# MarioPasc/MU-Diff

Hardware: AMD Instinct MI355X
Metric: 256x256 slices/sec (4-step dual-gen reverse) (higher is better)
Workload: dtype f32 (convs/attention: fp16 hi+lo split MFMA x3; 3x3 convs that fill the chip: fp16 hi.hi + e4m3 cross terms; fp32 accumulate); 1 GPU; BASELINE config 3 (BraTS-shaped test-split batches of 32; model and slice shapes of config 2): 4-step dual-generator sampling, 256x256, nf=64, ch_mult 1-2-4, 32 slices per GPU per step, batch-sharded over 1 GPU(s), weights replicated; batch=32, hipgraph=True

## Files before the change

include/mudiff_hip.h:

```cpp
#ifndef MUDIFF_HIP_H
#define MUDIFF_HIP_H

#include <stdint.h>

#ifdef __cplusplus
extern "C" {
#endif

#define MUD_OK 0
#define MUD_ERR_ARG 1
#define MUD_ERR_LAUNCH 2
#define MUD_ERR_UNSUPPORTED 3

#define MUD_ACT_NONE 0
#define MUD_ACT_SIGMOID 1
#define MUD_ACT_TANH 2
#define MUD_ACT_SILU 3
#define MUD_ACT_LRELU 4

#define MUD_PRO_NONE 0
#define MUD_PRO_AFFINE 1
#define MUD_PRO_AFFINE_SILU 2
#define MUD_PRO_LRELU 3

// ... 42 lines not shown
  const float* x;  int B, H, W, Cin, ldx;
  const void* w;   int64_t w_bstride;
  int ks, stride, pad;
  const float* pro_scale; const float* pro_shift; int pro_ld; int pro_mode;
  const float* bias;
  const float* bias2; int bias2_ld;
  const float* res; int ldr;
  float out_scale; int act;
  const float* emul; int ld_emul;
  const float* egate; int ld_egate;
  const float* eother; int ld_eother;
  float* out; int Cout, ldo;
  int sub2;
  double* stats; int stats_ld;
  int emul_cout;
  const double* gn_sums; int gn_sums_ld;
  int gn_G; float gn_eps; double gn_count;
  const float* gn_gamma; const float* gn_beta;
  int64_t gn_bstride;
  void* splitk_ws; int64_t splitk_ws_bytes;
  unsigned* splitk_counters; int splitk_ncounters;
  const void* skip_w; const float* skip_bias; float* skip_out; int skip_ldo;
  int prec; int w_exp;
} mud_conv_args;

int mud_conv2d_direct(const mud_conv_args* a, void* stream);

int64_t mud_packed_weight_bytes(int ks, int Cin, int Cout);
int mud_pack_weights(const float* src, int64_t s_tap, int64_t s_ci, int64_t s_co, int64_t src_bstride,
                     int ks, int Cin, int Cout, int nbatch, void* dst, void* stream);
int mud_pack_weights_prec(const float* src, int64_t s_tap, int64_t s_ci, int64_t s_co, int64_t src_bstride,
                          int ks, int Cin, int Cout, int nbatch, int prec, int w_exp, void* dst, void* stream);
int64_t mud_packed_weight_bytes_prec(int ks, int Cin, int Cout, int prec);
int mud_conv2d_mfma(const mud_conv_args* a, void* stream);
int mud_conv2d_mfma_prec_supported(const mud_conv_args* a, int prec);
int64_t mud_conv2d_mfma_splitk_bytes(const mud_conv_args* a);

typedef struct mud_census_args {
  const float* x; int B, H, W, C, ldx;
  const float* pro_scale; const float* pro_shift; int pro_ld; int pro_mode;
} mud_census_args;
typedef struct mud_census_out {
  uint64_t n, n_over, n_under, n_fp16_over, amax_bits;
} mud_census_out;
int mud_e4m3_census(const mud_census_args* a, mud_census_out* out, void* stream);

int mud_upfirdn2d(const float* in, int64_t planes, int H, int W, const float* kernel, int kh, int kw,
                  int up_x, int up_y, int down_x, int down_y, int pad_x0, int pad_x1, int pad_y0, int pad_y1,
                  float* out, void* stream);
int mud_fir_nhwc(const float* x, int B, int H, int W, int C, int ldx, const float* kernel_host, int kh, int kw,
                 int up, int down, int pad0, int pad1,
                 const float* pro_scale, const float* pro_shift, int pro_ld, int pro_mode,
                 float* out_h, int ldh, float* out_x, int ldxo, void* stream);

int mud_minibatch_stddev(const float* x, int B, int64_t hw, int C, int ld, int group, float* out, void* stream);

int mud_attention_supported(int C);
int64_t mud_attention_ws_bytes(int B, int N, int C);
int mud_attention(const float* qkv, int B, int N, int C, int ld, float scale, float* out, int ldo, void* ws, void* stream);
// ... 112 lines not shown
```

mu-diff_amd/backbones/layerspp.py:

```python
import numpy as np
import torch
import torch.nn as nn

from mudiff_hip import ops, precision
from mudiff_hip.ops import (ACT_NONE, ACT_SILU, INV_SQRT2, PRO_AFFINE, PRO_AFFINE_SILU, View)

from . import dense_layer, layers, up_or_down_sampling

conv1x1 = layers.ddpm_conv1x1
conv3x3 = layers.ddpm_conv3x3
NIN = layers.NIN
default_init = layers.default_init
dense = dense_layer.dense

FIR_K = (1, 3, 3, 1)


def _groups(c):
    return min(c // 4, 32)


def use_mfma(cin, cout):
    return cin % 4 == 0 and cin >= 8

# ... 268 lines not shown
            self.Conv_2 = conv1x1(in_ch, out_ch)
        self.skip_rescale, self.act, self.in_ch, self.out_ch = skip_rescale, act, in_ch, out_ch
        self.dropout = dropout

    def _prepare(self):
        d = dict(c0=ConvParam(self.Conv_0), c1=ConvParam(self.Conv_1))
        if hasattr(self, 'Conv_2'):
            d['c2'] = ConvParam(self.Conv_2)
            if self.up:
                d['c2'].bias = None
                d['c1'].bias = (self.Conv_1.bias.detach() + self.Conv_2.bias.detach()).contiguous()
        return d

    def run(self, x: View, style0, style1, tbias, out: View = None, arena=None):
        if self.dropout and self.training:
            raise NotImplementedError('dropout > 0 in training mode is not part of the inference path')
        p = self.prepared()
        fused = False
        gn0 = self.GroupNorm_0.scale_shift(x, style0)
        sc0, sh0 = (gn0, None) if isinstance(gn0, ops.LazyGN) else gn0
        if self.up:
            kk, up, down, pad = up_or_down_sampling.fir_params('up' if self.fir else 'naive_up', self.fir_kernel)
            h_in, _ = ops.fir_nhwc(x, kk, up, down, pad, pro=(sc0, sh0, PRO_AFFINE_SILU), want_h=True, want_x=False)
            x_skip, _ = ops.fir_nhwc(p['c2'](x), kk, up, down, pad)
            h = p['c0'](h_in, bias2=tbias, arena=arena)
        elif self.down:
            kk, up, down, pad = up_or_down_sampling.fir_params('down' if self.fir else 'naive_down', self.fir_kernel)
            h_in, x_skip = ops.fir_nhwc(x, kk, up, down, pad, pro=(sc0, sh0, PRO_AFFINE_SILU), want_h=True, want_x=True)
            h = p['c0'](h_in, bias2=tbias, arena=arena)
        else:
            x_skip = x
            fused = 'c2' in p and p['c0'].mfma and p['c2'].mfma and ops.fused_skip_ok(x, self.out_ch, PRO_AFFINE_SILU)
            if fused:
                x_skip = View.empty(x.B, x.H, x.W, self.out_ch, x.device)
                h = p['c0'](x, pro=(sc0, sh0, PRO_AFFINE_SILU), bias2=tbias, arena=arena, skip=(p['c2'].w, p['c2'].bias, x_skip))
            else:
                h = p['c0'](x, pro=(sc0, sh0, PRO_AFFINE_SILU), bias2=tbias, arena=arena)
        gn1 = self.GroupNorm_1.scale_shift(h, style1)
        sc1, sh1 = (gn1, None) if isinstance(gn1, ops.LazyGN) else gn1
        if 'c2' in p and not self.up and not fused:
            x_skip = p['c2'](x_skip)
        return p['c1'](h, pro=(sc1, sh1, PRO_AFFINE_SILU), res=x_skip, out_scale=INV_SQRT2 if self.skip_rescale else 1.0, out=out)

    def forward(self, x, temb=None, zemb=None):
        st0 = ops.dense(zemb, self.GroupNorm_0.style.weight.detach(), self.GroupNorm_0.style.bias.detach())
        st1 = ops.dense(zemb, self.GroupNorm_1.style.weight.detach(), self.GroupNorm_1.style.bias.detach())
        tb = None
        if temb is not None:
            tb = ops.dense(temb, self.Dense_0.weight.detach(), self.Dense_0.bias.detach(), act_in=ACT_SILU)
        return self.run(View.from_nchw(x), st0, st1, tb).to_nchw()


class ConvFeatBlock(nn.Module, _Prepared):

    def __init__(self, act, in_ch=None, out_ch=None, zemb_dim=256):
        super().__init__()
        self.conv1 = conv3x3(in_ch, out_ch)
        self.group_norm = GroupNorm_Conv(min(out_ch // 4, 32), out_ch)
        self.act = act
        self.conv2 = conv3x3(out_ch, out_ch)

    def _prepare(self):
        return dict(c1=ConvParam(self.conv1), c2=ConvParam(self.conv2))

    def run(self, x: View, out: View = None, arena=None):
# ... 124 lines not shown
```

mu-diff_amd/csrc/conv_direct.hip:

```cpp
#include "mud_common.h"
#include <stdlib.h>

template <int VO, int VI>
__global__ __launch_bounds__(256) void k_conv_direct(mud_conv_args a, int Ho, int Wo, int co_groups) {
  extern __shared__ __attribute__((aligned(16))) char smem_raw[];
  float* st_lds = (float*)smem_raw;
  const int b = blockIdx.y;
  if (a.stats) {
    for (int i = threadIdx.x; i < 2 * a.Cout; i += 256) st_lds[i] = 0.f;
    __syncthreads();
  }
  const unsigned total = (unsigned)Ho * (unsigned)Wo * (unsigned)co_groups;
  const unsigned nthreads = gridDim.x * blockDim.x;
  const unsigned stride = (nthreads / (unsigned)co_groups) * (unsigned)co_groups;
  const unsigned first = blockIdx.x * blockDim.x + threadIdx.x;
  const int cg = (int)(first % (unsigned)co_groups);
  float ssum[VO], ssq[VO];
#pragma unroll
  for (int j = 0; j < VO; ++j) ssum[j] = ssq[j] = 0.f;
  for (uint64_t idx64 = first; first < stride && idx64 < total; idx64 += stride) {
    const unsigned p = (unsigned)idx64 / (unsigned)co_groups;
    const int oy = (int)(p / (unsigned)Wo);
    const int ox = (int)(p - (unsigned)oy * (unsigned)Wo);
    const int co = cg * VO;
// ... 198 lines not shown
  }
  const int gy = ty0 + py, gx = tx0 + px;
  if (gy < a.H && gx < a.W) {
    const int64_t opix = ((int64_t)b * a.H + gy) * a.W + gx;
#pragma unroll
    for (int j = 0; j < COUT; ++j) {
      float v = acc[j];
      if (a.bias) v += a.bias[j];
      if (a.res) v += a.res[opix * a.ldr + j];
      a.out[opix * a.ldo + j] = mud_act(v * a.out_scale, a.act);
    }
  }
}

extern "C" int mud_conv2d_direct(const mud_conv_args* ap, void* stream) {
  MUD_REQUIRE(ap, "mud_conv2d_direct: null args");
  const mud_conv_args a = *ap;
  MUD_REQUIRE(a.x && a.w && a.out, "mud_conv2d_direct: null pointer");
  MUD_REQUIRE(a.B >= 0 && a.H > 0 && a.W > 0 && a.Cin > 0 && a.Cout > 0 && a.ks >= 1 && a.stride >= 1 && a.pad >= 0,
              "mud_conv2d_direct: bad sizes");
  MUD_REQUIRE(a.ldx >= a.Cin && a.ldo >= a.Cout, "mud_conv2d_direct: ld smaller than C");
  MUD_REQUIRE(a.pro_mode == MUD_PRO_NONE || a.pro_mode == MUD_PRO_LRELU || (a.pro_scale && a.pro_shift && a.pro_ld >= a.Cin), "mud_conv2d_direct: prologue arrays missing");
  MUD_REQUIRE(!a.res || a.ldr >= a.Cout, "mud_conv2d_direct: bad residual view");
  const int Ho = (a.H + 2 * a.pad - a.ks) / a.stride + 1, Wo = (a.W + 2 * a.pad - a.ks) / a.stride + 1;
  MUD_REQUIRE(Ho > 0 && Wo > 0, "mud_conv2d_direct: empty output");
  if (a.B == 0) return MUD_OK;
  const bool vo4 = a.Cout % 4 == 0 && a.ldo % 4 == 0 && mud_aligned16(a.out) && mud_aligned16(a.w) && (a.w_bstride % 16 == 0);
  const bool vi4 = a.Cin % 4 == 0 && a.ldx % 4 == 0 && mud_aligned16(a.x);
  const int co_groups = vo4 ? a.Cout / 4 : a.Cout;
  if (a.Cin == 1 && a.ks == 3 && ((a.stride == 1 && a.pad == 1) || (a.stride == 2 && a.pad == 0)) && vo4 && !a.emul && !a.egate && co_groups <= 256 && a.pro_mode == MUD_PRO_NONE && a.w_bstride == 0 &&
      (!a.res || (a.ldr % 4 == 0 && mud_aligned16(a.res))) && (!a.bias || mud_aligned16(a.bias)) &&
      (!a.bias2 || (a.bias2_ld % 4 == 0 && mud_aligned16(a.bias2)))) {
    MUD_REQUIRE(a.B <= 65535 && (!a.stats || a.stats_ld >= a.Cout), "mud_conv2d_direct: bad batch / stats view");
    const int spb = 256 / co_groups, strips_per_row = (int)mud_cdiv(Wo, HEAD_PIX);
    int64_t blocks = mud_cdiv((int64_t)Ho * strips_per_row, spb);
    if (blocks > 256 * 16) blocks = 256 * 16;
    if (a.stats) {
      static const int cap = getenv("MUD_HEAD_CAP") ? atoi(getenv("MUD_HEAD_CAP")) : 0;
      int64_t per_image = 2048 / a.B > 16 ? 2048 / a.B : 16;
      const int64_t lim = cap > 0 ? cap : (a.B == 1 ? 256 : 128);
      if (per_image > lim) per_image = lim;
      if (blocks > per_image) blocks = per_image;
    }
    if (a.stride == 1)
      hipLaunchKernelGGL(k_conv_head3x3<1>, dim3((int)blocks, a.B), dim3(256), a.stats ? 2 * a.Cout * sizeof(float) : 0, (hipStream_t)stream, a, co_groups,
                         strips_per_row, Ho, Wo);
// ... 38 lines not shown
```

mu-diff_amd/csrc/conv_mfma.hip:

```cpp
#include "mud_common.h"
#include <stdlib.h>
#include <type_traits>
#include <utility>

typedef int i32x4 __attribute__((ext_vector_type(4)));
typedef int i32x8 __attribute__((ext_vector_type(8)));
typedef _Float16 f16x4 __attribute__((ext_vector_type(4)));
typedef _Float16 f16x8 __attribute__((ext_vector_type(8)));

typedef mud_h16x4 h16x4;
typedef mud_h16x8 h16x8;
__device__ __forceinline__ int cm_e4m3x4(f32x4 v, float scale) {
  v = v * scale;
#pragma unroll
  for (int e = 0; e < 4; ++e) v[e] = __builtin_amdgcn_fmed3f(v[e], -448.0f, 448.0f);
  int p = __builtin_amdgcn_cvt_pk_fp8_f32(v[0], v[1], 0, false);
  return __builtin_amdgcn_cvt_pk_fp8_f32(v[2], v[3], p, true);
}
#define CM_BN 64
#define CM_BPLANE (CM_BN * 32)
#define CM_BSTEP (2 * CM_BPLANE)
#define CM_PIX 80
#define CM_GN_MAXC 1024
#define CM_GN_BYTES (2 * CM_GN_MAXC * 4)
// ... 312 lines not shown
        if (DUAL) acc2[m][n][i] = 0.f;
      }
  const int lane_a2 = ((wm * MT) * 32 + r) * 64 + ((hh ^ ((r >> 2) & 3)) << 4);

  if constexpr (X8) {
    if (q == 0) {
#pragma unroll
      for (int j = 0; j < G::NLOAD; ++j) {
        *(i32x4*)(smem + loff[j] + 64) = i32x4{0, 0, 0, 0};
        *(i32x4*)(smem + G::BUF + loff[j] + 64) = i32x4{0, 0, 0, 0};
      }
    }
  }
  dma_b(kc0 * G::NG);
  dma_b2(kc0);
  fetch_raw(kc0);

  const int emul_lim = a.emul_cout > 0 ? a.emul_cout : a.Cout;
  const bool vec = ((a.Cout | a.ldo | emul_lim | (a.res ? a.ldr : 0) | (a.emul ? a.ld_emul : 0) | (a.egate ? (a.ld_egate | a.ld_eother) : 0)) & 3) == 0 &&
                   mud_dev_aligned16(a.out) && (!a.res || mud_dev_aligned16(a.res)) && (!a.emul || mud_dev_aligned16(a.emul)) &&
                   (!a.egate || (mud_dev_aligned16(a.egate) && mud_dev_aligned16(a.eother)));
  const bool slab_mode = KS == 3 && nsplit > 1 && fin.counters != nullptr;
  const bool res_in_acc = !DUAL && KS == 3 && a.res != nullptr && !a.sub2 && nsplit == 1;
  if (res_in_acc) {
#pragma unroll
    for (int n = 0; n < 2; ++n) {
      const int co = (nt * WN + wn) * CM_BN + n * 32 + r;
#pragma unroll
      for (int m = 0; m < MT; ++m) {
        const int gy = ty0 + wm * MT + m;
#pragma unroll
        for (int reg = 0; reg < 16; ++reg) {
          const int gx = tx0 + (reg & 3) + 8 * (reg >> 2) + 4 * hh;
          const bool ok = gy < a.H && gx < a.W && co < a.Cout;
          acc[m][n][reg] = ok ? a.res[(((int64_t)b * a.H + gy) * a.W + gx) * a.ldr + co] : 0.f;
        }
      }
    }
  }

  if (gn_fold) {
    cm_gn_to_lds(a, b, tid, G::NT, (float*)(smem + G::GN_OFF), gn_c);
    __syncthreads();
  } else if (PRO == MUD_PRO_AFFINE || PRO == MUD_PRO_AFFINE_SILU) {
    float* sc_lds = (float*)(smem + G::GN_OFF);
    for (int c = tid; c < a.Cin; c += G::NT) {
      sc_lds[c] = psc[c];
// ... 831 lines not shown
      return MUD_ERR_LAUNCH;
    }
    attr_once.ok();
  }
  const int k16s = (int)mud_cdiv(a.Cin, 16), ntiles = (int)mud_cdiv(a.Cout, CM_BN * WN);
  const int lds = G::lds_bytes((PRO == MUD_PRO_AFFINE || PRO == MUD_PRO_AFFINE_SILU) ? a.Cin : 0);
  int tiles_x = 1;
  int64_t tiles;
  if (KS == 3) {
    tiles_x = (int)mud_cdiv(a.W, 32);
    tiles = (int64_t)tiles_x * mud_cdiv(a.H, WM * MT);
  } else {
    tiles = mud_cdiv((int64_t)a.H * a.W, G::P);
  }
  int64_t nblocks = tiles * ntiles * a.B;
  MUD_REQUIRE(nblocks <= 0x7fffffff, "mud_conv2d_mfma: grid too large");
  if constexpr (KS == 3) {
    const int64_t npix = (int64_t)a.B * a.H * a.W;
    int ns = 1;
    static const bool two_launches = getenv("MUD_CONV_SPLITK_2LAUNCH") != nullptr;
    const bool in_launch = !two_launches && a.splitk_counters && nblocks <= a.splitk_ncounters;
    if ((!DUAL || in_launch) && a.splitk_ws && mud_aligned16(a.splitk_ws) && cm_split_eligible(a)) ns = cm_splits(nblocks, k16s);
    if (ns > 1 && a.splitk_ws_bytes < cm_slab_bytes(ns, nblocks, 64 * WM * WN * 32 * MT * (DUAL ? 2 : 1))) ns = 1;
    if (ns > 1) {
      mud_conv_args p = a;
      p.out = (float*)a.splitk_ws;
      p.ldo = a.Cout;
      p.bias = p.bias2 = p.res = nullptr;
      p.out_scale = 1.0f;
      p.act = MUD_ACT_NONE;
      p.stats = nullptr;
      const int64_t stride = npix * a.Cout;
      if (in_launch) {
        hipLaunchKernelGGL((k_conv_mfma<KS, MT, WM, WN, PRO, DUAL, PREC>), dim3((unsigned)(nblocks * ns)), dim3(64 * WM * WN), lds, s, a, tiles_x,
                           (int)tiles, ntiles, k16s, (unsigned)(nblocks * ns), ns, (int64_t)0, CmFin{(float*)a.splitk_ws, a.splitk_counters});
        MUD_CHECK_LAUNCH("mud_conv2d_mfma(split-K, reduced in the launch)");
        return MUD_OK;
      }
      hipLaunchKernelGGL((k_conv_mfma<KS, MT, WM, WN, PRO, DUAL, PREC>), dim3((unsigned)(nblocks * ns)), dim3(64 * WM * WN), lds, s, p, tiles_x,
                         (int)tiles, ntiles, k16s, (unsigned)(nblocks * ns), ns, stride, CmFin{nullptr, nullptr});
      MUD_CHECK_LAUNCH("mud_conv2d_mfma(split-K)");
      const int64_t HW = (int64_t)a.H * a.W;
      int ppb = 32;
      while (ppb > 1 && HW % ppb) ppb >>= 1;
      hipLaunchKernelGGL(k_splitk_epilogue, dim3((unsigned)mud_cdiv(npix, ppb)), dim3(256), 0, s, a, (const float*)a.splitk_ws, ns, stride, a.Cout,
                         npix, ppb);
// ... 36 lines not shown
  if (!no8x1r && !a.skip_w && ntiles == 1 && a.Cin <= 64 && a.H >= 8 && blocks2 >= 512) v = CMV_8X1R, nb = blocks2;
  else if (ntiles % 2 == 0 && a.H >= 8 && blocks8 >= 256) v = CMV_8X2, nb = blocks8;
  else if (!no16 && a.H >= 16 && blocks16 >= 256) v = CMV_16X1, nb = blocks16;
  else if (blocks2 >= 512 && a.H >= 8) v = CMV_MT2, nb = blocks2;
  else v = CMV_MT1, nb = mud_cdiv(a.W, 32) * mud_cdiv(a.H, 4) * ntiles * a.B;
  if (blocks) *blocks = nb;
  return v;
}

extern "C" int64_t mud_conv2d_mfma_splitk_bytes(const mud_conv_args* ap) {
  if (!ap || ap->ks != 3 || ap->B <= 0 || ap->H <= 0 || ap->W <= 0 || ap->Cin <= 0 || ap->Cout <= 0 || !cm_split_eligible(*ap)) return 0;
  int64_t blocks = 0;
  int v = cm_variant3(*ap, &blocks);
  if (ap->skip_w) {
    if (!ap->splitk_counters) return 0;
    if (v != CMV_8X2 && v != CMV_16X1) {
      v = CMV_MT1;
      blocks = mud_cdiv(ap->W, 32) * mud_cdiv(ap->H, 4) * mud_cdiv(ap->Cout, CM_BN) * ap->B;
    }
  }
  const int ns = cm_splits(blocks, (int)mud_cdiv(ap->Cin, 16));
  const int tile_words = ((v == CMV_8X2 || v == CMV_16X1) ? 512 * 64 : v == CMV_MT2 ? 256 * 64 : v == CMV_8X1R ? 512 * 32 : 256 * 32) * (ap->skip_w ? 2 : 1);
  return ns > 1 ? cm_slab_bytes(ns, blocks, tile_words) : 0;
}

static bool cm_fp8x_built(const mud_conv_args& a) {
  if (a.ks != 3 || a.sub2 || (a.pro_mode != MUD_PRO_NONE && a.pro_mode != MUD_PRO_AFFINE_SILU)) return false;
  if (a.skip_w && a.pro_mode != MUD_PRO_AFFINE_SILU) return false;
  const int v = cm_variant3(a, nullptr);
  return v == CMV_8X2 || v == CMV_16X1 || v == CMV_8X1R;
}
extern "C" int mud_conv2d_mfma_prec_supported(const mud_conv_args* ap, int prec) {
  if (!ap || ap->B <= 0 || ap->H <= 0 || ap->W <= 0 || ap->Cin <= 0 || ap->Cout <= 0) return 0;
  if (prec == MUD_PREC_16X3) return ap->ks == 1 || ap->ks == 3;
  if (prec == MUD_PREC_16X1)
    return ap->ks == 3 && ap->pro_mode >= MUD_PRO_NONE && ap->pro_mode <= MUD_PRO_LRELU && (!ap->skip_w || ap->pro_mode == MUD_PRO_AFFINE_SILU);
  mud_conv_args a = *ap;
  a.prec = prec;
  return prec == MUD_PREC_FP8X && cm_fp8x_built(a);
}

extern "C" int mud_conv2d_mfma(const mud_conv_args* ap, void* stream) {
  MUD_REQUIRE(ap, "mud_conv2d_mfma: null args");
  mud_conv_args a = *ap;
  MUD_REQUIRE(a.x && a.w && a.out, "mud_conv2d_mfma: null pointer");
  MUD_REQUIRE((a.ks == 1 || a.ks == 3) && a.stride == 1 && a.pad == a.ks / 2, "mud_conv2d_mfma: only ks in {1,3}, stride 1, pad ks/2 (got ks=%d stride=%d pad=%d)", a.ks, a.stride, a.pad);
// ... 10 lines not shown
  if ((a.pro_mode == MUD_PRO_AFFINE || a.pro_mode == MUD_PRO_AFFINE_SILU) && a.gn_sums) {
    MUD_REQUIRE(a.Cin <= CM_GN_MAXC && a.gn_G > 0 && a.Cin % a.gn_G == 0 && a.gn_sums_ld >= a.Cin && a.gn_count > 0,
                "mud_conv2d_mfma: folded GroupNorm needs Cin <= %d, Cin %% gn_G == 0, gn_sums_ld >= Cin, gn_count > 0 (Cin=%d gn_G=%d)", CM_GN_MAXC, a.Cin, a.gn_G);
    MUD_REQUIRE((a.gn_gamma == nullptr) == (a.gn_beta == nullptr) && a.gn_bstride >= 0, "mud_conv2d_mfma: folded GroupNorm: gamma and beta come together");
    a.pro_scale = a.pro_shift = a.x;
    a.pro_ld = 0;
  } else if (a.pro_mode == MUD_PRO_AFFINE || a.pro_mode == MUD_PRO_AFFINE_SILU) {
    a.gn_sums = nullptr;
    MUD_REQUIRE(a.pro_scale && a.pro_shift && a.pro_ld >= a.Cin && a.pro_ld % 4 == 0 && mud_aligned16(a.pro_scale) && mud_aligned16(a.pro_shift),
                "mud_conv2d_mfma: prologue arrays missing or misaligned");
    MUD_REQUIRE(a.Cin <= CM_GN_MAXC, "mud_conv2d_mfma: a launch with prologue arrays takes Cin <= %d (the kernels keep them in LDS; Cin=%d)", CM_GN_MAXC, a.Cin);
  } else {
    a.pro_scale = a.pro_shift = a.x;
    a.pro_ld = 0;
    a.gn_sums = nullptr;
  }
  if (a.skip_w) {
    MUD_REQUIRE(a.ks == 3 && a.pro_mode == MUD_PRO_AFFINE_SILU && !a.res && !a.sub2 && !a.emul && !a.egate,
                "mud_conv2d_mfma: the fused skip conv needs ks == 3, the AFFINE_SILU prologue and a plain epilogue");
    MUD_REQUIRE(a.skip_out && a.Cin <= 512 && a.Cout % 4 == 0 && a.skip_ldo >= a.Cout && a.skip_ldo % 4 == 0 && a.ldo % 4 == 0 &&
                mud_aligned16(a.skip_w) && mud_aligned16(a.skip_out) && mud_aligned16(a.out),
                "mud_conv2d_mfma: fused skip conv needs Cin <= 512, Cout %% 4 == 0 and aligned float4 output rows (Cin=%d Cout=%d)", a.Cin, a.Cout);
  }
  MUD_REQUIRE(a.prec == MUD_PREC_16X3 || a.prec == MUD_PREC_FP8X || a.prec == MUD_PREC_16X1, "mud_conv2d_mfma: unknown arithmetic plan prec=%d", a.prec);
  MUD_REQUIRE(a.prec != MUD_PREC_16X1 || a.ks == 3, "mud_conv2d_mfma: MUD_PREC_16X1 is built for ks == 3 only (got ks=%d)", a.ks);
  MUD_REQUIRE(a.prec != MUD_PREC_FP8X || (cm_fp8x_built(a) && a.w_exp >= -100 && a.w_exp <= 100),
              "mud_conv2d_mfma: MUD_PREC_FP8X is not built for this launch (ask mud_conv2d_mfma_prec_supported first; the weights were packed for it and cannot be read by another plan)");
  if (a.B == 0) return MUD_OK;
  hipStream_t s = (hipStream_t)stream;
#ifdef MUD_EXPERIMENT_WS
  if (cm_ws_wanted(a)) return cm_ws_dispatch(a, s);
#endif
  if (a.prec == MUD_PREC_FP8X) {
    const int v8 = cm_variant3(a, nullptr);
    if (v8 == CMV_8X1R) return a.pro_mode == MUD_PRO_NONE ? cm_launch_pro<3, 1, 8, 1, MUD_PRO_NONE, false, MUD_PREC_FP8X>(a, s) : cm_launch_pro<3, 1, 8, 1, MUD_PRO_AFFINE_SILU, false, MUD_PREC_FP8X>(a, s);
    const bool x2 = v8 == CMV_8X2;
    if (a.skip_w) return x2 ? cm_launch_pro<3, 2, 4, 2, MUD_PRO_AFFINE_SILU, true, MUD_PREC_FP8X>(a, s) : cm_launch_pro<3, 2, 8, 1, MUD_PRO_AFFINE_SILU, true, MUD_PREC_FP8X>(a, s);
    if (a.pro_mode == MUD_PRO_NONE) return x2 ? cm_launch_pro<3, 2, 4, 2, MUD_PRO_NONE, false, MUD_PREC_FP8X>(a, s) : cm_launch_pro<3, 2, 8, 1, MUD_PRO_NONE, false, MUD_PREC_FP8X>(a, s);
    return x2 ? cm_launch_pro<3, 2, 4, 2, MUD_PRO_AFFINE_SILU, false, MUD_PREC_FP8X>(a, s) : cm_launch_pro<3, 2, 8, 1, MUD_PRO_AFFINE_SILU, false, MUD_PREC_FP8X>(a, s);
  }
  if (a.prec == MUD_PREC_16X1) {
    constexpr int P1 = MUD_PREC_16X1;
    if (a.skip_w) {
      switch (cm_variant3(a, nullptr)) {
        case CMV_8X2: return cm_launch_pro<3, 2, 4, 2, MUD_PRO_AFFINE_SILU, true, P1>(a, s);
        case CMV_16X1: return cm_launch_pro<3, 2, 8, 1, MUD_PRO_AFFINE_SILU, true, P1>(a, s);
// ... 36 lines not shown
```

mu-diff_amd/mudiff_hip/__init__.py:

```python
from __future__ import annotations

import ctypes as C
import os

import torch

_HERE = os.path.dirname(os.path.abspath(__file__))
_SHIPPED = os.path.join(_HERE, 'libmudiff_hip.so')
_LIB_PATH = os.environ.get('MUDIFF_HIP_LIB', _SHIPPED)
_lib = None
PREC_16X3, PREC_FP8X, PREC_16X1 = 0, 1, 2

ACT_NONE, ACT_SIGMOID, ACT_TANH, ACT_SILU, ACT_LRELU = 0, 1, 2, 3, 4
PRO_NONE, PRO_AFFINE, PRO_AFFINE_SILU, PRO_LRELU = 0, 1, 2, 3


class MudiffHipError(RuntimeError):
    pass


class ConvArgs(C.Structure):
    _fields_ = [
        ('x', C.c_void_p), ('B', C.c_int), ('H', C.c_int), ('W', C.c_int), ('Cin', C.c_int), ('ldx', C.c_int),
        ('w', C.c_void_p), ('w_bstride', C.c_int64),
        ('ks', C.c_int), ('stride', C.c_int), ('pad', C.c_int),
        ('pro_scale', C.c_void_p), ('pro_shift', C.c_void_p), ('pro_ld', C.c_int), ('pro_mode', C.c_int),
        ('bias', C.c_void_p),
        ('bias2', C.c_void_p), ('bias2_ld', C.c_int),
        ('res', C.c_void_p), ('ldr', C.c_int),
        ('out_scale', C.c_float), ('act', C.c_int),
        ('emul', C.c_void_p), ('ld_emul', C.c_int), ('egate', C.c_void_p), ('ld_egate', C.c_int), ('eother', C.c_void_p), ('ld_eother', C.c_int),
        ('out', C.c_void_p), ('Cout', C.c_int), ('ldo', C.c_int),
        ('sub2', C.c_int),
        ('stats', C.c_void_p), ('stats_ld', C.c_int),
        ('emul_cout', C.c_int),
        ('gn_sums', C.c_void_p), ('gn_sums_ld', C.c_int), ('gn_G', C.c_int), ('gn_eps', C.c_float), ('gn_count', C.c_double),
        ('gn_gamma', C.c_void_p), ('gn_beta', C.c_void_p), ('gn_bstride', C.c_int64),
        ('splitk_ws', C.c_void_p), ('splitk_ws_bytes', C.c_int64),
        ('splitk_counters', C.c_void_p), ('splitk_ncounters', C.c_int),
        ('skip_w', C.c_void_p), ('skip_bias', C.c_void_p), ('skip_out', C.c_void_p), ('skip_ldo', C.c_int),
        ('prec', C.c_int), ('w_exp', C.c_int),
    ]


MLP_MAX_LAYERS = 6


class MlpArgs(C.Structure):
    _fields_ = [
        ('x', C.c_void_p), ('ldx', C.c_int), ('B', C.c_int),
        ('nlayers', C.c_int), ('dims', C.c_int * (MLP_MAX_LAYERS + 1)),
        ('W', C.c_void_p * MLP_MAX_LAYERS), ('b', C.c_void_p * MLP_MAX_LAYERS),
        ('pixel_norm', C.c_int), ('act', C.c_int), ('act_last', C.c_int),
        ('out', C.c_void_p), ('ldo', C.c_int), ('maxdim', C.c_int),
    ]


class CensusArgs(C.Structure):
    _fields_ = [
        ('x', C.c_void_p), ('B', C.c_int), ('H', C.c_int), ('W', C.c_int), ('C', C.c_int), ('ldx', C.c_int),
        ('pro_scale', C.c_void_p), ('pro_shift', C.c_void_p), ('pro_ld', C.c_int), ('pro_mode', C.c_int),
    ]


# ... 15 lines not shown
_SIGNATURES = {
    'mud_version': (C.c_int, []),
    'mud_last_error': (C.c_char_p, []),
    'mud_build_flags': (C.c_char_p, []),
    'mud_posterior_sample': (_I, [_P, _P, _P, _P, _P, _P, _P, _P, _I, _P, _I, _L, _P]),
    'mud_q_sample': (_I, [_P, _P, _P, _I, _P, _P, _I, _P, _I, _L, _P]),
    'mud_timestep_embedding': (_I, [_P, _P, _I, _I, _F, _P]),
    'mud_pixel_norm': (_I, [_P, _P, _I, _I, _P]),
    'mud_dense': (_I, [_P, _I, _P, _P, _P, _I, _I, _I, _I, _I, _I, _P]),
    'mud_mlp_chain': (_I, [C.POINTER(MlpArgs), _P]),
    'mud_mlp_chains': (_I, [C.POINTER(MlpArgs), _I, _P]),
    'mud_gn_ws_bytes': (_L, [_I, _L, _I, _I]),
    'mud_gn_scale_shift': (_I, [_P, _I, _L, _I, _I, _I, _F, _P, _P, _L, _P, _P, _I, _P, _P, _P]),
    'mud_gn_scale_shift_from_sums': (_I, [_P, _I, _I, _I, _I, C.c_double, _F, _P, _P, _L, _P, _P, _I, _P]),
    'mud_channel_mean': (_I, [_P, _I, _L, _I, _I, _P, _I, _P, _P]),
    'mud_conv2d_direct': (_I, [C.POINTER(ConvArgs), _P]),
    'mud_packed_weight_bytes': (_L, [_I, _I, _I]),
    'mud_pack_weights': (_I, [_P, _L, _L, _L, _L, _I, _I, _I, _I, _P, _P]),
    'mud_pack_weights_prec': (_I, [_P, _L, _L, _L, _L, _I, _I, _I, _I, _I, _I, _P, _P]),
    'mud_packed_weight_bytes_prec': (_L, [_I, _I, _I, _I]),
    'mud_conv2d_mfma': (_I, [C.POINTER(ConvArgs), _P]),
    'mud_conv2d_mfma_prec_supported': (_I, [C.POINTER(ConvArgs), _I]),
    'mud_conv2d_mfma_splitk_bytes': (_L, [C.POINTER(ConvArgs)]),
    'mud_upfirdn2d': (_I, [_P, _L, _I, _I, _P, _I, _I, _I, _I, _I, _I, _I, _I, _I, _I, _P, _P]),
    'mud_fir_nhwc': (_I, [_P, _I, _I, _I, _I, _I, C.POINTER(C.c_float), _I, _I, _I, _I, _I, _I, _P, _P, _I, _I, _P, _I, _P, _I, _P]),
    'mud_minibatch_stddev': (_I, [_P, _I, _L, _I, _I, _I, _P, _P]),
    'mud_attention_supported': (_I, [_I]),
    'mud_attention_ws_bytes': (_L, [_I, _I, _I]),
    'mud_attention': (_I, [_P, _I, _I, _I, _I, _F, _P, _I, _P, _P]),
    'mud_softmax_rows': (_I, [_P, _L, _I, _I, _P]),
    'mud_mul': (_I, [_P, _I, _P, _I, _P, _I, _L, _I, _P]),
    'mud_gate_mix': (_I, [_P, _I, _P, _I, _P, _I, _P, _I, _I, _L, _I, _P, _I, _P]),
    'mud_fourier_embedding': (_I, [_P, _P, _P, _I, _I, _P]),
    'mud_resize_bilinear': (_I, [_P, _L, _I, _I, _I, _I, _P, _P]),
    'mud_affine_clamp': (_I, [_P, _L, _F, _F, _F, _F, _P, _P]),
    'mud_e4m3_census': (_I, [C.POINTER(CensusArgs), _P, _P]),
    'mud_value_range_ws_bytes': (_L, []),
    'mud_value_range': (_I, [_P, _L, _P, _L, _P, _P, _P]),
    'mud_quantize_u8': (_I, [_P, _L, _F, _F, _P, _P]),
    'mud_slice_metrics_ws_bytes': (_L, [_I, _I, _I]),
    'mud_slice_metrics_u8': (_I, [_P, _P, _I, _I, _I, _P, _P, _P, _P, _L, _P]),
    'mud_volume_metrics_ws_bytes': (_L, [_I, _I, _I, _I]),
    'mud_volume_metrics': (_I, [_P, _P, _P, _P, _I, _I, _I, _I, _P, _P, _L, _P]),
    'mud_lpips_packed_bytes': (_L, []),
    'mud_lpips_pack': (_I, [_P, _P, _P, _P, _P, _P]),
    'mud_lpips_ws_bytes': (_L, [_I, _I, _I]),
# ... 88 lines not shown
```

mu-diff_amd/mudiff_hip/ops.py:

```python
from __future__ import annotations

import collections
import ctypes as C
import math
import os

import numpy as np
import torch

from . import (ACT_LRELU, ACT_NONE, ACT_SIGMOID, ACT_SILU, ACT_TANH, PREC_16X1, PREC_16X3, PREC_FP8X, PRO_AFFINE, PRO_AFFINE_SILU, PRO_LRELU,
               PRO_NONE, ConvArgs, MudiffHipError, check, load, ptr, require_gpu)


DETERMINISTIC = os.environ.get('MUD_DETERMINISTIC', '0') == '1'


class StatsArena:

    def __init__(self, device, chunk_doubles=1 << 18):
        self.device, self.chunk = device, chunk_doubles
        self.buf, self.used = None, 0

    def take(self, B, C):
        if DETERMINISTIC:
# ... 309 lines not shown
        return _SPLITK_OWNED[-1]
    key = (device.index if device.index is not None else torch.cuda.current_device(), torch.cuda.current_stream(device).cuda_stream)
    buf = _SPLITK_COUNTERS.get(key)
    if buf is None:
        buf = _SPLITK_COUNTERS[key] = new_splitk_counters(device)
    return buf


def conv3x3_would_split_k(x: View, cout):
    a = ConvArgs()
    a.x, a.B, a.H, a.W, a.Cin, a.ldx, a.ks, a.stride, a.pad = x.ptr, x.B, x.H, x.W, x.C, x.ld, 3, 1, 1
    a.out, a.Cout, a.ldo = x.ptr, cout, (cout + 3) & ~3
    return load().mud_conv2d_mfma_splitk_bytes(C.byref(a)) > 0


FUSE_SKIP_SPLIT = os.environ.get('MUD_FUSE_SKIP_SPLIT', '1') != '0'


def fused_skip_ok(x: View, cout, pro_mode):
    return (FUSE_SKIP and pro_mode == PRO_AFFINE_SILU and x.C % 4 == 0 and 8 <= x.C <= 512 and cout % 4 == 0
            and (FUSE_SKIP_SPLIT or not conv3x3_would_split_k(x, cout)))


def resolve_pro(pro):
    if pro is not None and isinstance(pro[0], LazyGN):
        sc, sh = pro[0].tensors()
        return (sc, sh, pro[2])
    return pro


def channel_mean(x: View):
    lib = load()
    HW = x.H * x.W
    ws = _workspace(x.device, lib.mud_gn_ws_bytes(x.B, HW, x.C, x.C))
    out = torch.empty(x.B, x.C, device=x.device, dtype=torch.float32)
    _launch('channel_mean', x.device, lib.mud_channel_mean, x.ptr, x.B, HW, x.C, x.ld, ptr(out), x.C, ptr(ws), STREAM, nbytes=4.0 * x.npix * x.C)
    return out


def pack_weights(src, s_tap, s_ci, s_co, ks, Cin, Cout, nbatch=1, src_bstride=0, src_offset=0, prec=PREC_16X3, w_exp=0):
    lib = load()
    require_gpu(src)
    nbytes = lib.mud_packed_weight_bytes_prec(ks, Cin, Cout, prec)
    if nbytes < 0:
        raise MudiffHipError(f'pack_weights: plan {prec} has no packed form for ks={ks}')
    dst = torch.empty(nbatch, nbytes, device=src.device, dtype=torch.uint8)
# ... 59 lines not shown
    if skip:
        a.skip_w = x.ptr
    return bool(load().mud_conv2d_mfma_prec_supported(C.byref(a), prec))


def choose_prec(x: View, cout, pro_mode, *, skip=False, sub2=False, w_bstride=0):
    if PREC_PLAN == 'off' or w_bstride or x.C % 4:
        return PREC_16X3
    if PREC_PLAN == 'fp16':
        return PREC_16X1 if conv_prec_supported(x, cout, pro_mode, PREC_16X1, skip=skip, sub2=sub2) else PREC_16X3
    if PREC_PLAN != 'all' and not fp8x_pays(x.B, x.H, x.W, x.C, cout):
        return PREC_16X3
    return PREC_FP8X if conv_prec_supported(x, cout, pro_mode, PREC_FP8X, skip=skip, sub2=sub2) else PREC_16X3


Launch = collections.namedtuple('Launch', 'layer ks mfma prec shape sub2 skip pro')


RECORD = None


def conv(x: View, w, ks, Cout, *, mfma, stride=1, pad=None, pro=None, bias=None, bias2=None, res: View = None,
         out_scale=1.0, act=ACT_NONE, out: View = None, w_bstride=0, arena=None, sub2=False, emul: View = None, gate=None, emul_cout=0,
         skip=None, prec=PREC_16X3, w_exp=0, layer=None):
    if RECORD is not None:
        if torch.cuda.is_current_stream_capturing():
            raise RuntimeError('precision.launch_record() is eager only: the launch is being captured into a graph')
        RECORD.append(Launch(layer, ks, bool(mfma), prec, (x.B, x.H, x.W, x.C, Cout), bool(sub2), skip is not None,
                             PRO_NONE if pro is None else pro[2]))
    lib = load()
    pad = ks // 2 if pad is None else pad
    Ho = (x.H + 2 * pad - ks) // stride + 1
    Wo = (x.W + 2 * pad - ks) // stride + 1
    if sub2:
        assert mfma and ks == 3 and stride == 1 and x.H % 2 == 1 and x.W % 2 == 1
        Ho, Wo = x.H // 2, x.W // 2
    if out is None:
        out = View.empty(x.B, Ho, Wo, Cout, x.device, arena)
    assert (out.B, out.H, out.W, out.C) == (x.B, Ho, Wo, Cout), ((out.B, out.H, out.W, out.C), (x.B, Ho, Wo, Cout))
    a = ConvArgs()
    a.x, a.B, a.H, a.W, a.Cin, a.ldx = x.ptr, x.B, x.H, x.W, x.C, x.ld
    a.w, a.w_bstride = ptr(w), w_bstride
    a.ks, a.stride, a.pad = ks, stride, pad
    keep = None
    if pro is not None and isinstance(pro[0], LazyGN) and not (mfma and x.C <= 1024 and pro[0].x.stats is not None):
        pro = resolve_pro(pro)
    if pro is not None and pro[2] == PRO_LRELU:
        a.pro_mode = PRO_LRELU
    elif pro is not None and isinstance(pro[0], LazyGN):
        gn = keep = pro[0]
        assert gn.x.C == x.C and gn.x.B == x.B
        a.pro_mode = pro[2]
        a.gn_sums, a.gn_sums_ld, a.gn_G, a.gn_eps, a.gn_count = gn.x.stats_ptr, gn.x.stats.shape[1], gn.G, gn.eps, float(gn.x.H * gn.x.W)
        a.gn_gamma, a.gn_beta, a.gn_bstride = ptr(gn.gamma), ptr(gn.beta), gn.bstride
    elif pro is not None:
        sc, sh, mode = pro
        assert sc.shape == (x.B, x.C) and sc.stride(1) == 1 and sh.stride() == sc.stride()
        a.pro_scale, a.pro_shift, a.pro_ld, a.pro_mode = ptr(sc), ptr(sh), sc.stride(0), mode
    else:
        a.pro_mode = PRO_NONE
    if bias is not None:
        assert bias.numel() == Cout and bias.is_contiguous()
        a.bias = ptr(bias)
    if bias2 is not None:
        assert bias2.shape == (x.B, Cout) and bias2.stride(1) == 1
        a.bias2, a.bias2_ld = ptr(bias2), bias2.stride(0)
    if res is not None:
        assert (res.B, res.H, res.W, res.C) == (x.B, Ho, Wo, Cout)
        a.res, a.ldr = res.ptr, res.ld
    a.out_scale, a.act = out_scale, act
    a.sub2 = 1 if sub2 else 0
    if emul is not None:
        assert (emul.B, emul.H, emul.W, emul.C) == (x.B, Ho, Wo, emul_cout or Cout)
        a.emul, a.ld_emul, a.emul_cout = emul.ptr, emul.ld, emul_cout
    if gate is not None:
        gv, ov = gate
        assert (gv.B, gv.H, gv.W, gv.C) == (x.B, Ho, Wo, Cout) == (ov.B, ov.H, ov.W, ov.C)
        a.egate, a.ld_egate, a.eother, a.ld_eother = gv.ptr, gv.ld, ov.ptr, ov.ld
    a.out, a.Cout, a.ldo = out.ptr, Cout, out.ld
    a.prec, a.w_exp = prec, w_exp
    if out.stats is not None:
        a.stats, a.stats_ld = out.stats_ptr, out.stats.shape[1]
    skip_flops = 0.0
    if skip is not None:
        sw, sb, so = skip
        assert mfma and ks == 3 and res is None and (so.B, so.H, so.W, so.C) == (x.B, Ho, Wo, Cout)
        a.skip_w, a.skip_bias, a.skip_out, a.skip_ldo = ptr(sw), ptr(sb), so.ptr, so.ld
        skip_flops = 2.0 * x.B * Ho * Wo * Cout * x.C
    if mfma and ks == 3:
        cnt = splitk_counters(x.device)
        a.splitk_counters, a.splitk_ncounters = ptr(cnt), cnt.numel()
        nws = lib.mud_conv2d_mfma_splitk_bytes(C.byref(a))
        if nws > 0:
            keep = (keep, torch.empty(nws, device=x.device, dtype=torch.uint8))
            a.splitk_ws, a.splitk_ws_bytes = ptr(keep[1]), nws
    fn = lib.mud_conv2d_mfma if mfma else lib.mud_conv2d_direct
    name = (f'conv_mfma_k{ks}' if mfma else f'conv_direct_k{ks}') + {PREC_FP8X: '_fp8x', PREC_16X1: '_fp16'}.get(prec, '')
    flops = 2.0 * x.B * Ho * Wo * Cout * x.C * ks * ks + skip_flops
    nbytes = 4.0 * (x.npix * x.C + out.npix * Cout * ((2 if res is not None else 1) + (1 if skip is not None else 0))) + (w.numel() * w.element_size() if w_bstride == 0 else x.B * w_bstride)
    _launch(name, x.device, fn, C.byref(a), STREAM, flops=flops, nbytes=nbytes)
    return out


CENSUS_FIELDS = ('n', 'n_over', 'n_under', 'n_fp16_over', 'amax_bits')


def new_census_slot(device):
    return torch.zeros(len(CENSUS_FIELDS), device=device, dtype=torch.int64)


def e4m3_census(x: View, pro, out):
    from . import CensusArgs
# ... 561 lines not shown
```

Measured before the change: 102.1 slices/s.

## Fuse FIR 2x upsampling of the skip branch into the residual load of conv

In up-sampling ResNet blocks, the skip path's FIR upsample is no longer run as a separate kernel. The final 3x3 MFMA conv instead reads the low-resolution residual and applies the separable 4-tap up2 filter while it seeds its accumulators. This removes one full-resolution write and read plus a launch per up block. In exchange it adds scattered gather loads in the conv prologue and disables split-K for these convs.

```diff
diff --git a/include/mudiff_hip.h b/include/mudiff_hip.h
--- a/include/mudiff_hip.h
+++ b/include/mudiff_hip.h
@@ -88,6 +88,7 @@
   unsigned* splitk_counters; int splitk_ncounters;
   const void* skip_w; const float* skip_bias; float* skip_out; int skip_ldo;
   int prec; int w_exp;
+  int res_up2; float res_k[4];
 } mud_conv_args;
 
 int mud_conv2d_direct(const mud_conv_args* a, void* stream);
@@ -101,6 +102,7 @@
 int mud_conv2d_mfma(const mud_conv_args* a, void* stream);
 int mud_conv2d_mfma_prec_supported(const mud_conv_args* a, int prec);
 int64_t mud_conv2d_mfma_splitk_bytes(const mud_conv_args* a);
+int mud_conv2d_mfma_res_up2_supported(const mud_conv_args* a);
 
 typedef struct mud_census_args {
   const float* x; int B, H, W, C, ldx;
diff --git a/mu-diff_amd/backbones/layerspp.py b/mu-diff_amd/backbones/layerspp.py
--- a/mu-diff_amd/backbones/layerspp.py
+++ b/mu-diff_amd/backbones/layerspp.py
@@ -314,7 +314,10 @@
         if self.up:
             kk, up, down, pad = up_or_down_sampling.fir_params('up' if self.fir else 'naive_up', self.fir_kernel)
             h_in, _ = ops.fir_nhwc(x, kk, up, down, pad, pro=(sc0, sh0, PRO_AFFINE_SILU), want_h=True, want_x=False)
-            x_skip, _ = ops.fir_nhwc(p['c2'](x), kk, up, down, pad)
+            x_skip = p['c2'](x)
+            taps = ops.up2_taps(kk, up, down, pad) if p['c1'].mfma and ops.res_up2_ok(x.B, h_in.H, h_in.W, self.out_ch, self.out_ch) else None
+            if taps is None:
+                x_skip, _ = ops.fir_nhwc(x_skip, kk, up, down, pad)
             h = p['c0'](h_in, bias2=tbias, arena=arena)
         elif self.down:
             kk, up, down, pad = up_or_down_sampling.fir_params('down' if self.fir else 'naive_down', self.fir_kernel)
@@ -332,7 +335,8 @@
         sc1, sh1 = (gn1, None) if isinstance(gn1, ops.LazyGN) else gn1
         if 'c2' in p and not self.up and not fused:
             x_skip = p['c2'](x_skip)
-        return p['c1'](h, pro=(sc1, sh1, PRO_AFFINE_SILU), res=x_skip, out_scale=INV_SQRT2 if self.skip_rescale else 1.0, out=out)
+        kw = dict(res_up2=taps) if self.up and taps is not None else {}
+        return p['c1'](h, pro=(sc1, sh1, PRO_AFFINE_SILU), res=x_skip, out_scale=INV_SQRT2 if self.skip_rescale else 1.0, out=out, **kw)
 
     def forward(self, x, temb=None, zemb=None):
         st0 = ops.dense(zemb, self.GroupNorm_0.style.weight.detach(), self.GroupNorm_0.style.bias.detach())
diff --git a/mu-diff_amd/csrc/conv_direct.hip b/mu-diff_amd/csrc/conv_direct.hip
--- a/mu-diff_amd/csrc/conv_direct.hip
+++ b/mu-diff_amd/csrc/conv_direct.hip
@@ -244,6 +244,7 @@
   MUD_REQUIRE(a.ldx >= a.Cin && a.ldo >= a.Cout, "mud_conv2d_direct: ld smaller than C");
   MUD_REQUIRE(a.pro_mode == MUD_PRO_NONE || a.pro_mode == MUD_PRO_LRELU || (a.pro_scale && a.pro_shift && a.pro_ld >= a.Cin), "mud_conv2d_direct: prologue arrays missing");
   MUD_REQUIRE(!a.res || a.ldr >= a.Cout, "mud_conv2d_direct: bad residual view");
+  MUD_REQUIRE(!a.res_up2, "mud_conv2d_direct: res_up2 (a residual up-sampled on load) is built for mud_conv2d_mfma's 3x3 kernel only");
   const int Ho = (a.H + 2 * a.pad - a.ks) / a.stride + 1, Wo = (a.W + 2 * a.pad - a.ks) / a.stride + 1;
   MUD_REQUIRE(Ho > 0 && Wo > 0, "mud_conv2d_direct: empty output");
   if (a.B == 0) return MUD_OK;
diff --git a/mu-diff_amd/csrc/conv_mfma.hip b/mu-diff_amd/csrc/conv_mfma.hip
--- a/mu-diff_amd/csrc/conv_mfma.hip
+++ b/mu-diff_amd/csrc/conv_mfma.hip
@@ -358,7 +358,60 @@
                    (!a.egate || (mud_dev_aligned16(a.egate) && mud_dev_aligned16(a.eother)));
   const bool slab_mode = KS == 3 && nsplit > 1 && fin.counters != nullptr;
   const bool res_in_acc = !DUAL && KS == 3 && a.res != nullptr && !a.sub2 && nsplit == 1;
-  if (res_in_acc) {
+  constexpr bool UP2 = KS == 3 && !DUAL && PRO == MUD_PRO_AFFINE_SILU;
+  bool res_up2 = false;
+  if constexpr (UP2) res_up2 = res_in_acc && a.res_up2 != 0;
+  if (res_up2) {
+    if constexpr (UP2) {
+      const int Hl = a.H >> 1, Wl = a.W >> 1;
+      const float* rb = a.res + (int64_t)b * Hl * Wl * a.ldr;
+      const int jq = ((tx0 + 4 * hh) >> 1) - 1;
+      unsigned cmask = 0;
+#pragma unroll
+      for (int i = 0; i < 16; ++i) cmask |= (jq + i >= 0 && jq + i < Wl ? 1u : 0u) << i;
+      const int co0 = (nt * WN + wn) * CM_BN + r;
+      const float* rc = rb + (co0 < a.Cout ? co0 : 0);
+      const int dn = co0 + 32 < a.Cout ? 32 : 0;
+      unsigned cm[2] = {co0 < a.Cout ? cmask : 0u, co0 + 32 < a.Cout ? cmask : 0u};
+      asm volatile("" : "+v"(cm[0]), "+v"(cm[1]));
+#pragma unroll
+      for (int m = 0; m < MT; ++m) {
+        const int gy = ty0 + __builtin_amdgcn_readfirstlane(wm) * MT + m;
+        const int ay = gy & 1, y0 = (gy >> 1) - 1 + ay;
+        const float ky[2] = {(y0 >= 0 && y0 < Hl) ? (ay ? a.res_k[2] : a.res_k[3]) : 0.f, (y0 + 1 < Hl) ? (ay ? a.res_k[0] : a.res_k[1]) : 0.f};
+        const int yo[2] = {min(max(y0, 0), Hl - 1) * Wl, min(y0 + 1, Hl - 1) * Wl};
+#pragma unroll
+        for (int g4 = 0; g4 < 4; ++g4) {
+          float v[2][2][4];
+#pragma unroll
+          for (int ry = 0; ry < 2; ++ry)
+#pragma unroll
+            for (int cx = 0; cx < 4; ++cx) {
+              const float* pp = rc + (yo[ry] + min(max(jq + 4 * g4 + cx, 0), Wl - 1)) * a.ldr;
+              v[0][ry][cx] = pp[0];
+              v[1][ry][cx] = pp[dn];
+            }
+#pragma unroll
+          for (int n = 0; n < 2; ++n) {
+#pragma unroll
+            for (int ry = 0; ry < 2; ++ry)
+#pragma unroll
+              for (int cx = 0; cx < 4; ++cx) v[n][ry][cx] = (cm[n] & (1u << (4 * g4 + cx))) ? v[n][ry][cx] : 0.f;
+#pragma unroll
+            for (int e = 0; e < 4; ++e) {
+              const int ca = (e + 1) >> 1;
+              const float kx0 = (e & 1) ? a.res_k[2] : a.res_k[3], kx1 = (e & 1) ? a.res_k[0] : a.res_k[1];
+              float t = (ky[0] * kx0) * v[n][0][ca];
+              t = __builtin_fmaf(ky[0] * kx1, v[n][0][ca + 1], t);
+              t = __builtin_fmaf(ky[1] * kx0, v[n][1][ca], t);
+              t = __builtin_fmaf(ky[1] * kx1, v[n][1][ca + 1], t);
+              acc[m][n][g4 * 4 + e] = t;
+            }
+          }
+        }
+      }
+    }
+  } else if (res_in_acc) {
 #pragma unroll
     for (int n = 0; n < 2; ++n) {
       const int co = (nt * WN + wn) * CM_BN + n * 32 + r;
@@ -1236,6 +1289,7 @@
     const bool in_launch = !two_launches && a.splitk_counters && nblocks <= a.splitk_ncounters;
     if ((!DUAL || in_launch) && a.splitk_ws && mud_aligned16(a.splitk_ws) && cm_split_eligible(a)) ns = cm_splits(nblocks, k16s);
     if (ns > 1 && a.splitk_ws_bytes < cm_slab_bytes(ns, nblocks, 64 * WM * WN * 32 * MT * (DUAL ? 2 : 1))) ns = 1;
+    MUD_REQUIRE(ns == 1 || !a.res_up2, "mud_conv2d_mfma: res_up2 is not built for a launch split over K (ask mud_conv2d_mfma_res_up2_supported first)");
     if (ns > 1) {
       mud_conv_args p = a;
       p.out = (float*)a.splitk_ws;
@@ -1318,6 +1372,14 @@
   const int ns = cm_splits(blocks, (int)mud_cdiv(ap->Cin, 16));
   const int tile_words = ((v == CMV_8X2 || v == CMV_16X1) ? 512 * 64 : v == CMV_MT2 ? 256 * 64 : v == CMV_8X1R ? 512 * 32 : 256 * 32) * (ap->skip_w ? 2 : 1);
   return ns > 1 ? cm_slab_bytes(ns, blocks, tile_words) : 0;
+}
+
+extern "C" int mud_conv2d_mfma_res_up2_supported(const mud_conv_args* ap) {
+  if (!ap || ap->ks != 3 || ap->stride != 1 || ap->pad != 1 || ap->sub2 || ap->skip_w || ap->pro_mode != MUD_PRO_AFFINE_SILU) return 0;
+  if (ap->B <= 0 || ap->H <= 0 || ap->W <= 0 || ap->Cin <= 0 || ap->Cout <= 0 || (ap->H & 1) || (ap->W & 1)) return 0;
+  int64_t blocks = 0;
+  cm_variant3(*ap, &blocks);
+  return cm_splits(blocks, (int)mud_cdiv(ap->Cin, 16)) == 1;
 }
 
 static bool cm_fp8x_built(const mud_conv_args& a) {
@@ -1374,6 +1436,12 @@
                 mud_aligned16(a.skip_w) && mud_aligned16(a.skip_out) && mud_aligned16(a.out),
                 "mud_conv2d_mfma: fused skip conv needs Cin <= 512, Cout %% 4 == 0 and aligned float4 output rows (Cin=%d Cout=%d)", a.Cin, a.Cout);
   }
+  if (a.res_up2) {
+    MUD_REQUIRE(a.ks == 3 && a.res && !a.sub2 && !a.skip_w && (a.H & 1) == 0 && (a.W & 1) == 0 && a.pro_mode == MUD_PRO_AFFINE_SILU,
+                "mud_conv2d_mfma: res_up2 needs ks == 3, the AFFINE_SILU prologue, a residual, no sub2 / fused skip conv and even H, W (ks=%d H=%d W=%d sub2=%d pro_mode=%d)",
+                a.ks, a.H, a.W, a.sub2, a.pro_mode);
+    MUD_REQUIRE((int64_t)(a.H / 2) * (a.W / 2) * a.ldr < 0x7fffffffLL, "mud_conv2d_mfma: res_up2: one low-resolution image must stay below 2^31 elements");
+  }
   MUD_REQUIRE(a.prec == MUD_PREC_16X3 || a.prec == MUD_PREC_FP8X || a.prec == MUD_PREC_16X1, "mud_conv2d_mfma: unknown arithmetic plan prec=%d", a.prec);
   MUD_REQUIRE(a.prec != MUD_PREC_16X1 || a.ks == 3, "mud_conv2d_mfma: MUD_PREC_16X1 is built for ks == 3 only (got ks=%d)", a.ks);
   MUD_REQUIRE(a.prec != MUD_PREC_FP8X || (cm_fp8x_built(a) && a.w_exp >= -100 && a.w_exp <= 100),
diff --git a/mu-diff_amd/mudiff_hip/__init__.py b/mu-diff_amd/mudiff_hip/__init__.py
--- a/mu-diff_amd/mudiff_hip/__init__.py
+++ b/mu-diff_amd/mudiff_hip/__init__.py
@@ -40,6 +40,7 @@
         ('splitk_counters', C.c_void_p), ('splitk_ncounters', C.c_int),
         ('skip_w', C.c_void_p), ('skip_bias', C.c_void_p), ('skip_out', C.c_void_p), ('skip_ldo', C.c_int),
         ('prec', C.c_int), ('w_exp', C.c_int),
+        ('res_up2', C.c_int), ('res_k', C.c_float * 4),
     ]
 
 
@@ -101,6 +102,7 @@
     'mud_conv2d_mfma': (_I, [C.POINTER(ConvArgs), _P]),
     'mud_conv2d_mfma_prec_supported': (_I, [C.POINTER(ConvArgs), _I]),
     'mud_conv2d_mfma_splitk_bytes': (_L, [C.POINTER(ConvArgs)]),
+    'mud_conv2d_mfma_res_up2_supported': (_I, [C.POINTER(ConvArgs)]),
     'mud_upfirdn2d': (_I, [_P, _L, _I, _I, _P, _I, _I, _I, _I, _I, _I, _I, _I, _I, _I, _P, _P]),
     'mud_fir_nhwc': (_I, [_P, _I, _I, _I, _I, _I, C.POINTER(C.c_float), _I, _I, _I, _I, _I, _I, _P, _P, _I, _I, _P, _I, _P, _I, _P]),
     'mud_minibatch_stddev': (_I, [_P, _I, _L, _I, _I, _I, _P, _P]),
diff --git a/mu-diff_amd/mudiff_hip/ops.py b/mu-diff_amd/mudiff_hip/ops.py
--- a/mu-diff_amd/mudiff_hip/ops.py
+++ b/mu-diff_amd/mudiff_hip/ops.py
@@ -355,6 +355,25 @@
             and (FUSE_SKIP_SPLIT or not conv3x3_would_split_k(x, cout)))
 
 
+RES_UP2 = os.environ.get('MUD_RES_UP2', '1') != '0'
+
+
+def up2_taps(kernel2d, up, down, pad):
+    k = np.asarray(kernel2d, dtype=np.float32)
+    if k.shape != (4, 4) or (up, down, tuple(pad)) != (2, 1, (2, 1)) or not float(k.sum()) > 0.0:
+        return None
+    t = (k.sum(axis=1) / np.sqrt(k.sum())).astype(np.float32)
+    return tuple(float(v) for v in t) if np.array_equal(np.outer(t, t).astype(np.float32), k) else None
+
+
+def res_up2_ok(B, H, W, cin, cout):
+    if not RES_UP2 or cin % 4 or cout % 4:
+        return False
+    a = ConvArgs()
+    a.B, a.H, a.W, a.Cin, a.ldx, a.ks, a.stride, a.pad, a.Cout, a.ldo, a.pro_mode = B, H, W, cin, cin, 3, 1, 1, cout, cout, PRO_AFFINE_SILU
+    return bool(load().mud_conv2d_mfma_res_up2_supported(C.byref(a)))
+
+
 def resolve_pro(pro):
     if pro is not None and isinstance(pro[0], LazyGN):
         sc, sh = pro[0].tensors()
@@ -460,7 +479,7 @@
 
 def conv(x: View, w, ks, Cout, *, mfma, stride=1, pad=None, pro=None, bias=None, bias2=None, res: View = None,
          out_scale=1.0, act=ACT_NONE, out: View = None, w_bstride=0, arena=None, sub2=False, emul: View = None, gate=None, emul_cout=0,
-         skip=None, prec=PREC_16X3, w_exp=0, layer=None):
+         skip=None, prec=PREC_16X3, w_exp=0, layer=None, res_up2=None, split_k=True):
     if RECORD is not None:
         if torch.cuda.is_current_stream_capturing():
             raise RuntimeError('precision.launch_record() is eager only: the launch is being captured into a graph')
@@ -504,7 +523,11 @@
         assert bias2.shape == (x.B, Cout) and bias2.stride(1) == 1
         a.bias2, a.bias2_ld = ptr(bias2), bias2.stride(0)
     if res is not None:
-        assert (res.B, res.H, res.W, res.C) == (x.B, Ho, Wo, Cout)
+        if res_up2 is not None:
+            assert mfma and Ho % 2 == 0 and Wo % 2 == 0 and (res.B, res.H, res.W, res.C) == (x.B, Ho // 2, Wo // 2, Cout) and len(res_up2) == 4
+            a.res_up2, a.res_k = 1, (C.c_float * 4)(*res_up2)
+        else:
+            assert (res.B, res.H, res.W, res.C) == (x.B, Ho, Wo, Cout)
         a.res, a.ldr = res.ptr, res.ld
     a.out_scale, a.act = out_scale, act
     a.sub2 = 1 if sub2 else 0
@@ -525,7 +548,7 @@
         assert mfma and ks == 3 and res is None and (so.B, so.H, so.W, so.C) == (x.B, Ho, Wo, Cout)
         a.skip_w, a.skip_bias, a.skip_out, a.skip_ldo = ptr(sw), ptr(sb), so.ptr, so.ld
         skip_flops = 2.0 * x.B * Ho * Wo * Cout * x.C
-    if mfma and ks == 3:
+    if mfma and ks == 3 and split_k and res_up2 is None:
         cnt = splitk_counters(x.device)
         a.splitk_counters, a.splitk_ncounters = ptr(cnt), cnt.numel()
         nws = lib.mud_conv2d_mfma_splitk_bytes(C.byref(a))
```

Result: faster. 103.5 slices/s (median of 6 runs) (+1.3%).
